# Wangkkklll/GausPcc

Hardware: AMD Instinct MI355X
Metric: Mpoints/s encode+decode @1M anchors (higher is better)
Workload: dtype f32

## Files before the change

gauspcc_amd/_lib.py:

```python
import ctypes as C
import os

_HERE = os.path.dirname(os.path.abspath(__file__))
LIB_PATH = os.environ.get("GAUSPCC_LIB") or os.path.join(_HERE, "libgauspcc.so")

_lib = None


class GpccError(RuntimeError):
    def __init__(self, code, msg):
        super().__init__(f"libgauspcc error {code}: {msg}")
        self.code = code


class Stats(C.Structure):
    _fields_ = [
        ("num_points", C.c_int64),
        ("num_bytes", C.c_int64),
        ("num_levels", C.c_int32),
        ("flags", C.c_int32),
        ("level_nodes", C.c_int64 * 24),
        ("coded_nodes", C.c_int64),
        ("conv_pairs", C.c_int64),
        ("device_ms", C.c_double),
        ("ideal_bits", C.c_double),
    ]


class Profile(C.Structure):
    _fields_ = [("conv_ms", C.c_double), ("conv_launches", C.c_int64), ("conv_pair_jobs", C.c_int64),
                ("fused_ms", C.c_double), ("fused_launches", C.c_int64), ("fused_pair_jobs", C.c_int64)]


class Stage(C.Structure):
    _fields_ = [("name", C.c_char * 48), ("ms", C.c_double), ("bytes", C.c_double), ("brackets", C.c_int64), ("critical_ms", C.c_double)]


GSR_STATE_WORDS = 16
GPCC_TRAIN_STATE_WORDS = 256
GSR_ALLOC = C.CFUNCTYPE(C.c_void_p, C.c_void_p, C.c_size_t)

EXPORTS = [
    "gpcc_last_error", "gpcc_version", "gpcc_ctx_create", "gpcc_ctx_destroy", "gpcc_ctx_bytes", "gpcc_ctx_set_container_version", "gpcc_raster_order", "gpcc_voxelise",
    "gpcc_model_create", "gpcc_model_destroy", "gpcc_encode", "gpcc_decode", "gpcc_decode_to", "gpcc_encode_batch", "gpcc_decode_batch", "gpcc_sort_zyx",
    "gpcc_build_octree", "gpcc_conv3d", "gpcc_head_cdf", "gpcc_rc_encode", "gpcc_rc_decode", "gpcc_memcpy_d2d",
    "gpcc_profile_enable", "gpcc_profile_get", "gpcc_profile_stages", "gpcc_debug_trace_enable", "gpcc_debug_trace_get", "gpcc_debug_capture", "gpcc_debug_capture_get", "gpcc_debug_exclusive_scan", "gpcc_debug_launches", "gpcc_device_error_check",
    "gsac_calculate_cdf", "gsac_encode", "gsac_decode", "gsac_encode_u16", "gsac_decode_u16", "gsac_encode_const", "gsac_decode_const", "gsac_host_encode_u16", "gsac_host_decode_u16", "gsac_host_encode_f32", "gsac_host_decode_f32", "gpcc_write_files", "gpcc_read_files", "gsac_encode_gaussian", "gsac_decode_gaussian", "gsac_encode_gaussian_mixed", "gsac_decode_gaussian_mixed", "gsac_calculate_cdf_mixed", "gsac_encode_gaussian_slices", "gsac_decode_gaussian_slices", "gsac_encode_gaussian_mixed_slices", "gsac_decode_gaussian_mixed_slices", "gshac_mlp2", "gshac_mlp2_act", "gsge_forward", "gsge_forward_train", "gsge_backward", "gsr_visible_filter", "gsr_forward", "gsr_forward_train", "gsr_backward", "gsnn_generate", "gsnn_forward_train", "gsnn_backward",
    "gpcc_train_frame", "gpcc_train_frame_nodes", "gpcc_train_weights", "gpcc_train_conv", "gpcc_train_wgrad",
    "gpcc_knn", "gpcc_scatter_max", "gpcc_grow_voxels",
    "gsr_ssim_forward", "gsr_ssim_backward",
    "gsac_rate_forward", "gsac_rate_backward",
]


def lib():
    global _lib
    if _lib is not None:
        return _lib
    if not os.path.exists(LIB_PATH):
        raise ImportError(
            f"{LIB_PATH} is missing: build it with `python -c 'import __graft_entry__ as g; g.build()'` "
            "(make -C gauspcc_amd/csrc). gauspcc_amd has no CPU fallback."
        )
    import torch

    L = C.CDLL(LIB_PATH)
    vp, i64, i32, u16 = C.c_void_p, C.c_int64, C.c_int, C.c_uint16
    L.gpcc_last_error.restype = C.c_char_p
    L.gpcc_ctx_create.argtypes = [i32, C.POINTER(vp)]
    L.gpcc_ctx_destroy.argtypes = [vp]
    L.gpcc_ctx_destroy.restype = None
    L.gpcc_ctx_bytes.argtypes = [vp, C.POINTER(i64), C.POINTER(i64)]
    L.gpcc_ctx_set_container_version.argtypes = [vp, i32]
    L.gpcc_raster_order.argtypes = [vp, vp, i32, i64, vp, vp]
    L.gpcc_voxelise.argtypes = [vp, vp, i32, i64, C.c_double, C.c_double, C.c_double, i32, vp, vp]
    L.gpcc_model_create.argtypes = [vp, i32, i32, vp, C.POINTER(vp)]
    L.gpcc_model_destroy.argtypes = [vp]
    L.gpcc_model_destroy.restype = None
    L.gpcc_encode.argtypes = [vp, vp, vp, i64, i32, u16, C.POINTER(vp), C.POINTER(i64), C.POINTER(Stats), vp]
    L.gpcc_decode.argtypes = [vp, vp, vp, i64, C.POINTER(vp), C.POINTER(i64), C.POINTER(u16), C.POINTER(Stats), vp]
    L.gpcc_encode_batch.argtypes = [vp, vp, C.POINTER(vp), C.POINTER(i64), i32, i32, C.POINTER(u16), C.POINTER(vp), C.POINTER(i64), C.POINTER(Stats), C.POINTER(i32), vp]
    L.gpcc_decode_batch.argtypes = [vp, vp, C.POINTER(vp), C.POINTER(i64), i32, C.POINTER(vp), C.POINTER(i64), C.POINTER(i64), C.POINTER(u16), C.POINTER(Stats), C.POINTER(i32), vp]
    L.gpcc_decode_to.argtypes = [vp, vp, vp, i64, vp, i64, C.POINTER(i64), C.POINTER(u16), C.POINTER(Stats), vp]
    L.gpcc_sort_zyx.argtypes = [vp, vp, i64, vp, vp]
    L.gpcc_build_octree.argtypes = [vp, vp, i64, C.POINTER(i32), C.POINTER(i64), vp, vp, i64, vp]
    L.gpcc_conv3d.argtypes = [vp, vp, i64, i32, i32, vp, vp, vp, i32, vp, C.POINTER(i64), vp]
    L.gpcc_head_cdf.argtypes = [vp, vp, i64, i32, i32, vp, vp, vp, vp, vp, vp, vp]
    L.gpcc_rc_encode.argtypes = [vp, vp, i32, vp, i64, i32, C.POINTER(vp), C.POINTER(i64), vp]
    L.gpcc_rc_decode.argtypes = [vp, vp, i32, vp, i64, i64, i32, vp, vp]
    L.gpcc_memcpy_d2d.argtypes = [vp, vp, vp, i64, vp]
    L.gpcc_profile_enable.argtypes = [vp, i32]
    L.gpcc_debug_trace_enable.argtypes = [vp, i32]
    L.gpcc_debug_trace_get.argtypes = [vp, vp, vp, i32]
    L.gpcc_debug_capture.argtypes = [vp, i32]
    L.gpcc_debug_capture_get.restype = C.c_longlong
    L.gpcc_debug_capture_get.argtypes = [vp, i32, vp, C.c_longlong]
    L.gpcc_debug_exclusive_scan.argtypes = [vp, vp, vp, vp, vp, i64, vp, vp]
    L.gpcc_debug_launches.argtypes = [i32]
    L.gpcc_device_error_check.argtypes = [vp]
    L.gpcc_debug_launches.restype = C.c_longlong
    L.gpcc_profile_get.argtypes = [vp, C.POINTER(Profile)]
    L.gpcc_profile_stages.argtypes = [vp, C.POINTER(Stage), i32, C.POINTER(i32)]
    L.gsac_calculate_cdf.argtypes = [vp, vp, vp, vp, i64, i32, i32, vp, vp]
    L.gsac_encode.argtypes = [vp, vp, vp, i32, i64, i32, C.POINTER(vp), C.POINTER(i64), C.POINTER(vp), C.POINTER(i64), vp]
    L.gsac_decode.argtypes = [vp, vp, vp, i64, vp, i32, i64, i32, vp, vp]
    L.gsac_encode_u16.argtypes = L.gsac_encode.argtypes
    L.gsac_decode_u16.argtypes = L.gsac_decode.argtypes
    L.gsac_encode_const.argtypes = L.gsac_encode.argtypes
    L.gsac_decode_const.argtypes = L.gsac_decode.argtypes
    L.gsac_host_encode_u16.argtypes = [vp, vp, i64, i32, vp, i64, C.POINTER(i64)]
    L.gsac_host_decode_u16.argtypes = [vp, vp, i64, i64, i32, vp]
    L.gsac_host_encode_f32.argtypes = L.gsac_host_encode_u16.argtypes
    L.gsac_host_decode_f32.argtypes = L.gsac_host_decode_u16.argtypes
    L.gpcc_write_files.argtypes = [vp, vp, vp, i32, i32]
    L.gpcc_read_files.argtypes = [vp, i32, i32, C.POINTER(vp), vp]
    fp = C.POINTER(C.c_float)
    L.gsac_encode_gaussian.argtypes = [vp, vp, vp, vp, vp, i64, i32, fp, fp, C.POINTER(vp), C.POINTER(i64), C.POINTER(vp), C.POINTER(i64), vp]
    L.gsac_decode_gaussian.argtypes = [vp, vp, vp, vp, i64, C.c_float, C.c_float, vp, i64, vp, i32, vp, vp]
    L.gsac_encode_gaussian_mixed.argtypes = [vp, vp, vp, vp, vp, i32, vp, i64, i32, fp, fp, C.POINTER(vp), C.POINTER(i64), C.POINTER(vp), C.POINTER(i64), vp]
    L.gsac_decode_gaussian_mixed.argtypes = [vp, vp, vp, vp, i32, vp, i64, C.c_float, C.c_float, vp, i64, vp, i32, vp, vp]
    L.gsac_calculate_cdf_mixed.argtypes = [vp, vp, vp, vp, i32, vp, i64, i32, i32, vp, vp]
    L.gsac_encode_gaussian_slices.argtypes = [vp, vp, vp, vp, vp, vp, i32, i32, vp, vp, C.POINTER(vp), C.POINTER(i64), C.POINTER(vp), C.POINTER(i64), vp]
    L.gsac_decode_gaussian_slices.argtypes = [vp, vp, vp, vp, vp, i32, vp, vp, vp, i64, vp, i32, vp, vp]
    L.gshac_mlp2.argtypes = [vp, vp, vp, vp, vp, vp, i64, i32, i32, i32, vp, vp]
    L.gshac_mlp2_act.argtypes = [vp, vp, vp, vp, vp, vp, i64, i32, i32, i32, i32, C.c_float, vp, vp]
    L.gsac_encode_gaussian_mixed_slices.argtypes = [vp, vp, vp, vp, vp, i32, vp, vp, i32, i32, vp, vp, C.POINTER(vp), C.POINTER(i64), C.POINTER(vp), C.POINTER(i64), vp]
    L.gsac_decode_gaussian_mixed_slices.argtypes = [vp, vp, vp, vp, i32, vp, vp, i32, vp, vp, vp, i64, vp, i32, vp, vp]
    L.gsge_forward.argtypes = [vp, vp, vp, vp, vp, vp, i64, i32, i32, i32, i32, vp, vp, vp]
    L.gsge_forward_train.argtypes = [vp, vp, vp, vp, vp, vp, i64, i32, i32, i32, i32, vp, vp, vp, vp]
    L.gsge_backward.argtypes = [vp, vp, vp, vp, vp, vp, i64, vp, vp, i64, i32, i32, i32, i32, vp, vp, GSR_ALLOC, vp, vp]
    f32 = C.c_float
    L.gsr_visible_filter.argtypes = [vp, i32, i32, i32, vp, vp, f32, vp, vp, vp, vp, f32, f32, i32, vp, vp]
    L.gsr_forward.argtypes = [vp, i32, vp, i32, i32, vp, vp, vp, vp, f32, vp, vp, vp, vp, f32, f32, i32, vp, vp, C.POINTER(i64), vp]
    L.gsr_forward_train.argtypes = [vp, i32, vp, i32, i32, vp, vp, vp, vp, f32, vp, vp, vp, vp, f32, f32, i32, vp, vp, GSR_ALLOC, vp,
                                    C.POINTER(C.c_uint64), C.POINTER(i64), vp]
    L.gsr_backward.argtypes = [vp, C.POINTER(C.c_uint64), i32, vp, i32, i32, vp, vp, vp, vp, f32, vp, vp, vp, vp, f32, f32, vp, vp, GSR_ALLOC, vp,
                               vp, vp, vp, vp, vp, vp, vp, vp]
    L.gsnn_generate.argtypes = [vp, i64, vp, i32, i32, vp, vp, vp, vp, vp, vp, vp, vp, vp, vp, vp, vp, C.POINTER(i64), vp]
    L.gsnn_forward_train.argtypes = [vp, i64, i32, i32, vp, vp, vp, vp, vp, vp, vp, i32, vp, vp, vp, vp, vp, vp, vp, GSR_ALLOC, vp, C.POINTER(vp),
                                     C.POINTER(i64), vp]
    L.gsnn_backward.argtypes = [vp, i64, i32, i32, vp, vp, vp, vp, vp, vp, vp, i32, vp, vp, vp, vp, vp, vp, vp, vp, vp, vp, vp, vp, vp, GSR_ALLOC, vp, vp]
    st = C.POINTER(C.c_uint64)
    L.gpcc_train_frame.argtypes = [vp, vp, i64, i32, GSR_ALLOC, vp, st, C.POINTER(i32), C.POINTER(i64), vp]
    L.gpcc_train_frame_nodes.argtypes = [vp, st, vp, vp, vp, vp, vp]
    L.gpcc_train_weights.argtypes = [vp, vp, i32, i32, i32, vp, vp]
    L.gpcc_train_conv.argtypes = [vp, st, i32, vp, vp, vp, i32, vp, vp]
    L.gpcc_train_wgrad.argtypes = [vp, st, i32, vp, vp, GSR_ALLOC, vp, vp, vp]
    L.gpcc_knn.argtypes = [vp, vp, i64, i32, vp, vp, vp, GSR_ALLOC, vp, vp]
    L.gpcc_scatter_max.argtypes = [vp, vp, vp, i64, i64, i64, i32, vp, vp, GSR_ALLOC, vp, vp]
    L.gpcc_grow_voxels.argtypes = [vp, vp, i64, vp, vp, i64, i64, vp, i64, f32, f32, C.POINTER(i64), GSR_ALLOC, vp, vp]
    L.gsr_ssim_forward.argtypes = [vp, vp, vp, i64, i64, i64, i64, i32, fp, i32, vp, vp, vp, C.c_double, vp, i32, GSR_ALLOC, vp, vp]
    L.gsr_ssim_backward.argtypes = [vp, vp, vp, i64, i64, i64, i64, i32, fp, i32, vp, i32, vp, f32, vp, f32, vp, vp, vp]
    pp, ip, f64 = C.POINTER(vp), C.POINTER(i32), C.c_double
# ... 10 lines not shown
```

gauspcc_amd/csrc/api.hip:

```cpp
#include <algorithm>

#include "fused.hpp"
#include "network.hpp"
#include "octree.hpp"
#include "primitives.hpp"
#include "rangecoder_dev.hpp"

using namespace gpcc;

namespace gpcc {
thread_local char g_err[512] = "";
thread_local long long g_launches = 0;
}

extern "C" const char *gpcc_last_error(void) { return gpcc::g_err; }
extern "C" int gpcc_version(void) { return 100; }

extern "C" int gpcc_ctx_create(int device, gpcc_ctx **out)
{
    if (!out) return fail(GPCC_ERR_ARG, "null argument");
    int count = 0;
    HIP_TRY(hipGetDeviceCount(&count));
    if (device < 0 || device >= count) return fail(GPCC_ERR_ARG, "device %d not present (%d visible)", device, count);
    HIP_TRY(hipSetDevice(device));
    hipDeviceProp_t prop;
    HIP_TRY(hipGetDeviceProperties(&prop, device));
    if (strncmp(prop.gcnArchName, "gfx950", 6) != 0) return fail(GPCC_ERR_ARG, "libgauspcc is built for gfx950 (MI355X); device %d is %s", device, prop.gcnArchName);
    gpcc_ctx *c = new gpcc_ctx();
    c->device = device;
    *out = c;
    return GPCC_OK;
}

extern "C" void gpcc_ctx_destroy(gpcc_ctx *c)
{
    if (!c) return;
    (void)hipSetDevice(c->device);
    for (hipEvent_t e : c->prof.pool) (void)hipEventDestroy(e);
    if (c->side) { (void)hipStreamSynchronize(c->side); (void)hipStreamDestroy(c->side); (void)hipStreamSynchronize(c->xfer); (void)hipStreamDestroy(c->xfer); (void)hipEventDestroy(c->ev_main); (void)hipEventDestroy(c->ev_side); (void)hipEventDestroy(c->ev_bytes); (void)hipEventDestroy(c->ev_tables); }
    if (c->arena.base) (void)hipFree(c->arena.base);
    if (c->conv_products) (void)hipFree(c->conv_products);
    fused_ctx_release(c);
    if (c->fused_state) (void)hipFree(c->fused_state);
    for (auto &ss : c->scan_states) if (ss.status) (void)hipFree(ss.status);
    if (c->dev_err) (void)hipHostFree(c->dev_err);
    if (c->hbytes.p) (void)hipHostFree(c->hbytes.p);
    if (c->dbg_dev) (void)hipFree(c->dbg_dev);
    for (auto &e : c->dbg_caps) if (e.dev) (void)hipFree(e.dev);
    if (c->hstage.p) (void)hipHostFree(c->hstage.p);
    if (c->hcoder.p) (void)hipHostFree(c->hcoder.p);
    if (c->hbatch.p) (void)hipHostFree(c->hbatch.p);
    delete c;
}

extern "C" int gpcc_device_error_check(gpcc_ctx *ctx)
{
    if (!ctx) return fail(GPCC_ERR_ARG, "null argument");
    return device_error_check(ctx);
}

extern "C" long long gpcc_debug_launches(int reset)
{
    const long long v = gpcc::g_launches;
    if (reset) gpcc::g_launches = 0;
    return v;
}

extern "C" int gpcc_ctx_set_container_version(gpcc_ctx *c, int version)
{
    if (!c) return fail(GPCC_ERR_ARG, "null argument");
    if (version != 3 && version != 4) return fail(GPCC_ERR_ARG, "container version must be 3 or 4");
    c->container_version = version;
    return GPCC_OK;
}

extern "C" int gpcc_ctx_bytes(const gpcc_ctx *c, int64_t *device_bytes, int64_t *pinned_bytes)
{
    if (!c) return fail(GPCC_ERR_ARG, "null argument");
    size_t d = c->arena.cap + c->conv_products_cap * sizeof(float) + (c->dbg_dev ? 8 * (size_t)4096 : 0);
    d += c->scan_states.size() * (8 * (size_t)65536 + 256);
    if (c->fused_state) d += 2 * 3456 + 128;
    for (const auto &e : c->dbg_caps) d += e.cap;
    if (device_bytes) *device_bytes = (int64_t)d;
    if (pinned_bytes) *pinned_bytes = (int64_t)(c->hbytes.cap + c->hstage.cap + c->hbatch.cap + c->hcoder.cap);
    return GPCC_OK;
}

namespace gpcc {
constexpr int DBG_MAX = 4096;
__global__ __launch_bounds__(256) void k_dbg_sum(const uint32_t *__restrict__ p, size_t words, unsigned long long *__restrict__ out)
{
    unsigned long long a = 0;
    for (size_t i = (size_t)blockIdx.x * 256 + threadIdx.x; i < words; i += (size_t)gridDim.x * 256) a += (unsigned long long)p[i] * (2ull * i + 1ull);
    atomicAdd(out, a);
}
int dbg_mark(gpcc_ctx *ctx, hipStream_t st, int tag, const void *p, size_t bytes)
{
    if (!ctx || !ctx->dbg_on || (int)ctx->dbg_tags.size() >= DBG_MAX) return GPCC_OK;
    const size_t words = bytes / 4;
    unsigned long long *slot = ctx->dbg_dev + ctx->dbg_tags.size();
    HIP_TRY(hipMemsetAsync(slot, 0, 8, st));
    if (words) k_dbg_sum<<<(unsigned)std::min<size_t>(1024, (words + 255) / 256), 256, 0, st>>>(static_cast<const uint32_t *>(p), words, slot);
    LAUNCH_CHECK();
    ctx->dbg_tags.push_back(tag);
    if (ctx->dbg_capture_tag_mod >= 0 && tag % 100 == ctx->dbg_capture_tag_mod && bytes) {
        gpcc_ctx::DbgCap *c = nullptr;
        for (auto &e : ctx->dbg_caps) if (e.tag == tag) c = &e;
        if (!c) { ctx->dbg_caps.push_back(gpcc_ctx::DbgCap{tag, nullptr, 0, 0}); c = &ctx->dbg_caps.back(); }
        if (c->cap < bytes) {
            if (c->dev) HIP_TRY(hipFree(c->dev));
            c->dev = nullptr; c->cap = 0;
            HIP_TRY(hipMalloc(&c->dev, bytes));
            c->cap = bytes;
        }
        c->bytes = bytes;
        HIP_TRY(hipMemcpyAsync(c->dev, p, bytes, hipMemcpyDeviceToDevice, st));
    }
    return GPCC_OK;
// ... 608 lines not shown
```

gauspcc_amd/csrc/codec.hip:

```cpp
#include <algorithm>
#include <chrono>

#include <functional>
#include "hostcoder.hpp"
#include "codec_shared.hpp"
#include "container.hpp"
#include "rangecoder_dev.hpp"

using namespace gpcc;

namespace {

constexpr int ENC_RETRY_SMALLER_CHUNKS = -1000;
constexpr int DEC_RETRY_UNFUSED = -1001;

__global__ __launch_bounds__(256) void k_set_pos(SetLevels S, int64_t nC, uint32_t *__restrict__ pos_out, uint32_t *__restrict__ slots_out)
{
    const int64_t i = (int64_t)blockIdx.x * 256 + threadIdx.x;
    if (i >= nC) return;
    int d = 1;
    for (int q = 2; q < S.L; ++q) d = i >= (int64_t)S.cbase[q] ? q : d;
    pos_out[i] = S.lohi_base[d] + rc_interleaved(S.m2r[d][i - S.cbase[d]], S.clog[d], S.nch[d]);
    slots_out[i] = S.slots[d];
}
// ... 712 lines not shown
    }
    return GPCC_OK;
}

}

static size_t arena_scaled(size_t want)
{
    static const double scale = [] { const char *e = getenv("GAUSPCC_ARENA_SCALE"); const double v = e ? atof(e) : 1.0; return v > 0.0 ? v : 1.0; }();
    return scale == 1.0 ? want : std::max<size_t>((size_t)((double)want * scale), (size_t)1 << 20);
}

extern "C" int gpcc_encode(gpcc_ctx *ctx, const gpcc_model *m, const int32_t *xyz_dev, int64_t n, int chunk_log2, uint16_t posq_f16,
                           const uint8_t **bytes_out, int64_t *nbytes_out, gpcc_stats *stats, void *stream)
{
    if (!ctx || !m || !xyz_dev || !bytes_out || !nbytes_out) return fail(GPCC_ERR_ARG, "null argument");
    if (chunk_log2 != 0 && (chunk_log2 < 6 || chunk_log2 > 14)) return fail(GPCC_ERR_ARG, "chunk_log2 must be 0 or 6..14");
    HIP_TRY(hipSetDevice(ctx->device));
    hipStream_t st = (hipStream_t)stream;
    const auto t0 = std::chrono::steady_clock::now();
    size_t want = arena_scaled(arena_estimate(n, m->K));
    int rc = GPCC_OK;
    for (int attempt = 0; attempt < 6; ++attempt) {
        GP_TRY(ctx->arena.reserve(want));
        rc = encode_body(ctx, m, xyz_dev, n, chunk_log2, posq_f16, bytes_out, nbytes_out, stats, st);
        if (rc == ENC_RETRY_SMALLER_CHUNKS) {
            HIP_TRY(hipStreamSynchronize(st));
            if (chunk_log2 <= 6) { rc = GPCC_ERR_ARG; break; }
            chunk_log2 -= 1; attempt -= 1;
            continue;
        }
        if (rc != GPCC_ERR_NOMEM) break;
        HIP_TRY(hipStreamSynchronize(st));
        want *= 2;
    }
    if (rc == GPCC_OK && stats) stats->device_ms = std::chrono::duration<double, std::milli>(std::chrono::steady_clock::now() - t0).count();
    if (const int de = device_error_check(ctx)) rc = de;
    return rc;
}

static int decode_entry(gpcc_ctx *ctx, const gpcc_model *m, const uint8_t *bytes, int64_t nbytes, const int32_t **xyz_dev_out,
                        int64_t *n_out, uint16_t *posq_f16_out, gpcc_stats *stats, void *stream, int32_t *out_user, int64_t out_cap)
{
    HIP_TRY(hipSetDevice(ctx->device));
    hipStream_t st = (hipStream_t)stream;
    const auto t0 = std::chrono::steady_clock::now();
    size_t want = arena_estimate(std::max<int64_t>(nbytes, 1 << 16), m->K);
    int64_t nodes = 0, nmax = 0, npts = 0;
    const int pre = container_precheck(bytes, nbytes, &nodes, &nmax, &npts);
    if (pre < 0) return pre;
    if (pre > 0) {
        const int L = bytes[6];
        want = (size_t)nmax * 2600 + (size_t)nodes * (size_t)(4 * 125 + m->K * 81 / 16 + 96) + (size_t)npts * 32 + (size_t)nbytes + ((size_t)48 << 20);
        if (fused_enabled()) {
            int64_t nf = 0;
            for (int d = 0; d < L; ++d) { const int64_t v = get32(bytes + 8 + 4 * d); if (fused_level_ok(v, m->k)) nf = std::max(nf, v); }
            want += (size_t)nf * (size_t)m->K * (128 + 10 + 9) + ((size_t)4 << 20);
        }
    }
    want = arena_scaled(want);
    ctx->fused_note_decode();
    int rc = GPCC_OK;
    const int32_t *xyz = nullptr;
    for (int attempt = 0; attempt < 6; ++attempt) {
        GP_TRY(ctx->arena.reserve(want));
        rc = decode_body(ctx, m, bytes, nbytes, &xyz, n_out, posq_f16_out, stats, st, out_user, out_cap);
        if (rc == DEC_RETRY_UNFUSED) {
            static const bool loud = getenv("GAUSPCC_FUSED_QUIET") == nullptr;
            if (loud) fprintf(stderr, "[gauspcc] a persistent small-level launch timed out on device %d; the launch-per-layer path serves this context's next %d decodes\n", ctx->device, ctx->fused_rearm_after);
            attempt -= 1;
            continue;
        }
        if (rc != GPCC_ERR_NOMEM) break;
        HIP_TRY(hipStreamSynchronize(st));
        want *= 2;
    }
    if (rc == GPCC_OK && xyz_dev_out) *xyz_dev_out = xyz;
    if (rc == GPCC_OK && stats) stats->device_ms = std::chrono::duration<double, std::milli>(std::chrono::steady_clock::now() - t0).count();
    if (const int de = device_error_check(ctx)) rc = de;
    return rc;
}

extern "C" int gpcc_decode(gpcc_ctx *ctx, const gpcc_model *m, const uint8_t *bytes, int64_t nbytes, const int32_t **xyz_dev_out,
                           int64_t *n_out, uint16_t *posq_f16_out, gpcc_stats *stats, void *stream)
{
    if (!ctx || !m || !bytes || !xyz_dev_out || !n_out || !posq_f16_out) return fail(GPCC_ERR_ARG, "null argument");
    return decode_entry(ctx, m, bytes, nbytes, xyz_dev_out, n_out, posq_f16_out, stats, stream, nullptr, 0);
}

extern "C" int gpcc_decode_to(gpcc_ctx *ctx, const gpcc_model *m, const uint8_t *bytes, int64_t nbytes, int32_t *xyz_dev, int64_t capacity_points,
                              int64_t *n_out, uint16_t *posq_f16_out, gpcc_stats *stats, void *stream)
{
    if (!ctx || !m || !bytes || !xyz_dev || capacity_points < 0 || !n_out || !posq_f16_out) return fail(GPCC_ERR_ARG, "null argument");
    return decode_entry(ctx, m, bytes, nbytes, nullptr, n_out, posq_f16_out, stats, stream, xyz_dev, capacity_points);
}
```

gauspcc_amd/csrc/codec_batch.hip:

```cpp
#include <algorithm>
#include <chrono>
#include <functional>

#include "codec_shared.hpp"
#include "container.hpp"
#include "forest.hpp"
#include "rangecoder_dev.hpp"

using namespace gpcc;

extern "C" int gpcc_encode(gpcc_ctx *ctx, const gpcc_model *m, const int32_t *xyz_dev, int64_t n, int chunk_log2, uint16_t posq_f16, const uint8_t **bytes_out, int64_t *nbytes_out,
                           gpcc_stats *stats, void *stream);
extern "C" int gpcc_decode_to(gpcc_ctx *ctx, const gpcc_model *m, const uint8_t *bytes, int64_t nbytes, int32_t *xyz_dev, int64_t capacity_points, int64_t *n_out,
                              uint16_t *posq_f16_out, gpcc_stats *stats, void *stream);

namespace {

constexpr int BATCH_SOLO = -2001;
constexpr int BATCH_RETRY_UNFUSED = -2002;

struct FPosArgs {
    int L;
    uint32_t cbase[MAXLV];
    const uint32_t *m2r[MAXLV];
// ... 807 lines not shown
            if (r1 != GPCC_OK) {
                char msg[400]; snprintf(msg, sizeof msg, "%s", g_err);
                return fail(r1, "scene %d: %s", q, msg);
            }
            offsets_out[q] = (int64_t)blob.size();
            blob.insert(blob.end(), b, b + nb);
            if (stats) stats[q] = s1;
        }
        offsets_out[nscenes] = (int64_t)blob.size();
        GP_TRY(ctx->hbytes.reserve(blob.size() + 16));
        memcpy(ctx->hbytes.p, blob.data(), blob.size());
        *bytes_out = ctx->hbytes.p;
        rc = GPCC_OK;
    }
    if (rc == GPCC_OK && stats) stats[0].device_ms = std::chrono::duration<double, std::milli>(std::chrono::steady_clock::now() - t0).count();
    if (const int de = device_error_check(ctx)) rc = de;
    return rc;
}

extern "C" int gpcc_decode_batch(gpcc_ctx *ctx, const gpcc_model *m, const uint8_t *const *bytes, const int64_t *nbytes, int nscenes, int32_t *const *xyz_dev,
                                 const int64_t *capacity_points, int64_t *n_out, uint16_t *posq_f16_out, gpcc_stats *stats, int *batched_out, void *stream)
{
    if (!ctx || !m || !bytes || !nbytes || !xyz_dev || !capacity_points || !n_out || !posq_f16_out || nscenes < 1) return fail(GPCC_ERR_ARG, "null argument");
    for (int q = 0; q < nscenes; ++q) if (!bytes[q] || !xyz_dev[q] || capacity_points[q] < 0 || nbytes[q] < 0) return fail(GPCC_ERR_ARG, "scene %d: null argument", q);
    HIP_TRY(hipSetDevice(ctx->device));
    hipStream_t st = (hipStream_t)stream;
    const auto t0 = std::chrono::steady_clock::now();
    int rc = BATCH_SOLO;
    if (batched_out) *batched_out = 0;
    static const bool never = env_int("GAUSPCC_BATCH", 1) == 0;
    if (nscenes <= FOREST_MAX_SCENES && !never) {
        int64_t nodes = 0, nmax_sum[MAXLV] = {0}, total_bytes = 0, npts = 0;
        bool ok = true;
        for (int q = 0; q < nscenes && ok; ++q) {
            const uint8_t *b = bytes[q];
            total_bytes += nbytes[q];
            if (!(nbytes[q] >= 8 && b[0] == 0xFF && b[1] == 0xFF && b[6] >= 1 && b[6] <= 21 && nbytes[q] >= 12 + 4 * (int64_t)b[6])) { ok = false; break; }
            const int L = b[6];
            int64_t prev = 0, mine = 0;
            for (int d = 0; d < L; ++d) {
                const int64_t v = get32(b + 8 + 4 * d);
                if (v <= 0 || (d == 0 ? v >= 64 : v > 8 * prev)) { ok = false; break; }
                mine += v; nmax_sum[d] += v; prev = v;
            }
            if (!ok) break;
            const int64_t np = get32(b + 8 + 4 * L);
            if (np < 1 || np > 8 * prev || mine > (nbytes[q] << 13)) { ok = false; break; }
            nodes += mine; npts += np;
        }
        if (ok) {
            ctx->fused_note_decode();
            int64_t nmax = 0;
            for (int d = 0; d < MAXLV; ++d) nmax = std::max(nmax, nmax_sum[d]);
            size_t want = arena_scaled_b((size_t)nmax * 2700 + (size_t)nodes * (size_t)(4 * 125 + m->K * 81 / 16 + 96) + (size_t)npts * 32 + (size_t)total_bytes + (size_t)nscenes * 65536 + ((size_t)48 << 20));
            if (fused_enabled()) {
                int64_t nf = 0;
                for (int d = 0; d < MAXLV; ++d) if (nmax_sum[d] > 0 && fused_level_ok(nmax_sum[d], m->k)) nf = std::max(nf, nmax_sum[d]);
                want += (size_t)nf * (size_t)m->K * (128 + 10 + 9) + ((size_t)4 << 20);
            }
            for (int attempt = 0; attempt < 6; ++attempt) {
                GP_TRY(ctx->arena.reserve(want));
                rc = decode_batch_body(ctx, m, bytes, nbytes, nscenes, xyz_dev, capacity_points, n_out, posq_f16_out, stats, st);
                if (rc == BATCH_RETRY_UNFUSED) {
                    static const bool loud = getenv("GAUSPCC_FUSED_QUIET") == nullptr;
                    if (loud) fprintf(stderr, "[gauspcc] a persistent small-level launch timed out on device %d; the launch-per-layer path serves this context's next %d decodes\n", ctx->device, ctx->fused_rearm_after);
                    attempt -= 1;
                    continue;
                }
                if (rc != GPCC_ERR_NOMEM) break;
                HIP_TRY(hipStreamSynchronize(st));
                want *= 2;
            }
            if (rc == GPCC_OK && batched_out) *batched_out = 1;
        }
    }
    if (rc == BATCH_SOLO) {
        HIP_TRY(hipStreamSynchronize(st));
        for (int q = 0; q < nscenes; ++q) {
            gpcc_stats s1; memset(&s1, 0, sizeof s1);
            const int r1 = gpcc_decode_to(ctx, m, bytes[q], nbytes[q], xyz_dev[q], capacity_points[q], &n_out[q], &posq_f16_out[q], &s1, stream);
            if (r1 != GPCC_OK) {
                char msg[400]; snprintf(msg, sizeof msg, "%s", g_err);
                return fail(r1, "scene %d: %s", q, msg);
            }
            if (stats) stats[q] = s1;
        }
        rc = GPCC_OK;
    }
    if (rc == GPCC_OK && stats) stats[0].device_ms = std::chrono::duration<double, std::milli>(std::chrono::steady_clock::now() - t0).count();
    if (const int de = device_error_check(ctx)) rc = de;
    return rc;
}
```

gauspcc_amd/csrc/network.hpp:

```cpp
#pragma once
#include "common.hpp"

struct gpcc_model {
    int C = 32, k = 5, K = 125;
    float *slab = nullptr;
    const float *prior_emb = nullptr;
    const float *conv[18] = {0};
    const float *temb = nullptr;
    const float *hw1[4] = {0}, *hb1[4] = {0}, *hw2[4] = {0}, *hb2[4] = {0};
    const float *hfrag[4] = {0};
    const float *semb[3] = {0};
};

namespace gpcc {

__host__ __device__ __forceinline__ int phys_of(int c)
{
    const int kk = c >> 2, g = c & 3;
    return kk < 4 ? 4 * g + kk : 16 + 4 * g + (kk - 4);
}
__host__ __device__ __forceinline__ int logical_of(int p)
{
    const int kk = 4 * (p >> 4) + (p & 3), g = (p & 15) >> 2;
    return 4 * kk + g;
// ... 17 lines not shown
                for (int lane = 0; lane < 64; ++lane)
                    for (int r = 0; r < 4; ++r) {
                        const int m = lane & 15;
                        out[((((size_t)o * 2 + hh) * 2 + q) * 64 + lane) * 4 + r] = W[((size_t)o * 32 + (4 * (4 * q + r) + (lane >> 4))) * 32 + 16 * hh + 4 * (m & 3) + (m >> 2)];
                    }
}

constexpr int STAGE_M[4] = {2, 2, 4, 16};

struct ConvJob {
    const float *in;
    const float *w;
    const float *res;
    float *out;
};
struct ConvBatch { ConvJob job[4]; int C = 0; };

constexpr int CONV_R_MAX = 255;
constexpr int CONV_HDR_PAD = 48;
struct ConvTiles {
    int32_t *tj = nullptr;
    uint8_t *tr = nullptr;
    uint32_t *toc = nullptr;
    uint32_t *first = nullptr;
    uint32_t *order = nullptr;
    int64_t nblk = 0;
    int R = CONV_R_MAX;
    int H = CONV_R_MAX;
    int K = 0;
    int paired = 0;
    const uint8_t *pflag = nullptr;
    int nlv = 0;
    uint32_t lv_blk0[MAXLV + 1] = {0};
    uint32_t lv_row0[MAXLV] = {0};
    uint32_t lv_rows[MAXLV] = {0};
};
int conv_pick_rows(int64_t n, int k = 5);
bool conv_is_coop(int64_t n, int R);
int conv_pick_height(int64_t n, int R);

struct Level;
struct TileLevel { const Level *lv; const Level *par; const int32_t *cell_par; int32_t *cell_own; };
struct TilePool {
    int32_t *tj = nullptr; uint8_t *tr = nullptr; uint32_t *toc = nullptr; uint32_t *first = nullptr;
    int64_t nblk = 0;
    int R = 0, H = 0, K = 0, nlv = 0, paired = 0;
    uint8_t *pflag = nullptr;
    uint32_t lv_blk0[MAXLV + 1] = {0}, lv_rows[MAXLV] = {0};
    double alg_bytes = 0.0;
};
int cell_map_entries(int k);
int tiles_build(gpcc_ctx *ctx, hipStream_t st, const TileLevel *lv, int nlv, int k, int R, int H, TilePool *pool, unsigned long long *pairs_dev);
int tiles_dense_map(hipStream_t st, const Level *par, const int32_t *cell_par, const Level *chi, int32_t *cell_own, int k, int32_t *nbr, uint16_t *rk, uint32_t *rowcnt);
int tiles_view(gpcc_ctx *ctx, hipStream_t st, const TilePool &pool, int l0, int l1, const int64_t *row_base, ConvTiles *T);

int sparse_conv(gpcc_ctx *ctx, int level, hipStream_t st, const ConvBatch &jobs, int njobs, const ConvTiles &T, int64_t n, int relu);
int conv_chain_begin(gpcc_ctx *ctx, hipStream_t st);
int conv_chain_end(gpcc_ctx *ctx, hipStream_t st);
int prof_collect(gpcc_ctx *ctx, const unsigned long long *pairs_per_level, int nlevels);

int embed_occ(hipStream_t st, const float *emb, const uint8_t *occ, int64_t n, float *out, int C = 32);
int child_features(hipStream_t st, const float *F, const uint32_t *parent, const uint64_t *rkey_c, const float *temb, int64_t n, float *out, int C = 32);
int stage_inputs_gt(hipStream_t st, const float *X, const float *const emb[3], const uint8_t *occ, int64_t n, float *const out[3], int C = 32);
int stage_input_dec(hipStream_t st, const float *X, const float *emb, const uint8_t *const sym_r[3], const uint32_t *m2r, int stage, int64_t n, float *out, int C = 32);

constexpr int HEAD_FRAG_FLOATS = 1024 + 512 + 32 + 16;
struct HeadArgs {
    const float *x; int64_t n; int stage_m;
    const float *w1, *b1, *w2, *b2;
    const float *frag;
    const uint32_t *m2r; const uint8_t *occ; int stage;
    uint32_t *lohi; uint16_t *cdf; float *prob; int mode;
    int chunk_log2; uint32_t nch;
    const uint32_t *pos; const uint32_t *slots;
    double *bits;
    int C;
};
int head_cdf(hipStream_t st, const HeadArgs &a);

int assemble_occ(hipStream_t st, const uint8_t *const sym_r[4], const uint32_t *m2r, int64_t n, uint8_t *occ);

int any_embed_occ(hipStream_t st, const float *emb, const uint8_t *occ, int64_t n, float *out, int C);
int any_child_features(hipStream_t st, const float *F, const uint32_t *parent, const uint64_t *rkey_c, const float *temb, int64_t n, float *out, int C);
int any_stage_inputs_gt(hipStream_t st, const float *X, const float *const emb[3], const uint8_t *occ, int64_t n, float *const out[3], int C);
int any_stage_input_dec(hipStream_t st, const float *X, const float *emb, const uint8_t *const sym_r[3], const uint32_t *m2r, int stage, int64_t n, float *out, int C);
int any_sparse_conv(hipStream_t st, const ConvBatch &jobs, int njobs, const ConvTiles &T, int64_t n, int relu, int C);
int any_head_cdf(hipStream_t st, const HeadArgs &a, int C);

int rows_permute(hipStream_t st, const float *in, float *out, int64_t n, int to_physical);

}
```

gauspcc_amd/csrc/tiles.hip:

```cpp
#include "network.hpp"
#include "octree.hpp"
#include "primitives.hpp"

namespace gpcc {

namespace {

struct LevelTilesArgs {
    const uint64_t *rkey_c; const uint32_t *parent_c; int64_t nc;
    const int32_t *cell_p; int64_t np; const uint8_t *occ_p; const uint32_t *cstart_p;
    int H;
    int paired;
    uint8_t *pflag;
    uint32_t blk0;
    int32_t *cell_c;
    uint32_t *per_block;
    unsigned long long *pairs;
    uint8_t *cnt_oq;
    const uint32_t *first;
    int32_t *tj; uint8_t *tr; uint32_t *toc;
    int32_t *nbr; uint16_t *rk; uint32_t *rowcnt;
};

struct WaveMap {
// ... 328 lines not shown
        uint32_t inc = nt;
#pragma unroll
        for (int d = 1; d < 64; d <<= 1) {
            const uint32_t v = (uint32_t)__shfl_up((int)inc, d, 64);
            if (lane >= d) inc += v;
        }
        const uint32_t tb = carry + inc - nt;
        for (uint32_t i = 0; i < nt; ++i) toc[tb + i] = (uint32_t)o | ((tot > 16u * i ? min(16u, tot - 16u * i) : 0u) << 16);
        for (uint32_t p = tot; p < nt * 16u; ++p) { tj[(size_t)tb * 16 + p] = 0; tr[(size_t)tb * 16 + p] = 0; }
        carry += (uint32_t)__shfl((int)inc, 63, 64);
    }
}

template <int KS, bool FILL>
int launch_level(hipStream_t st, const LevelTilesArgs &a, bool tail)
{
    const int H = a.H;
    const bool multi = H == 16 || H == 32;
    const int nq = H > 64 ? (H + 63) / 64 : 1;
    const unsigned grid = multi ? (unsigned)cdiv(a.nc, 64) : (unsigned)(cdiv(a.nc, H) * nq);
    if (nq > 1) k_chunk_tiles<KS, FILL, true><<<grid, 64, 0, st>>>(a);
    else k_chunk_tiles<KS, FILL, false><<<grid, 64, 0, st>>>(a);
    LAUNCH_CHECK();
    if (nq > 1 && tail) {
        const int nblk = (int)cdiv(a.nc, H);
        if (!FILL) k_block_sum<<<(unsigned)cdiv(nblk, 4), 256, 0, st>>>(a.cnt_oq, a.blk0, nblk, KS * KS * KS, a.per_block, a.paired, a.pflag);
        else k_tile_words<<<(unsigned)cdiv(nblk, 4), 256, 0, st>>>(a.cnt_oq, a.first, a.blk0, nblk, KS * KS * KS, a.tj, a.tr, a.toc, a.pflag);
        LAUNCH_CHECK();
    }
    return GPCC_OK;
}

template <bool FILL>
int run_level(hipStream_t st, const Level *par, const int32_t *cell_par, const Level *chi, int k, LevelTilesArgs a, bool tail = true)
{
    a.rkey_c = chi->rkey; a.parent_c = chi->parent; a.nc = chi->n;
    if (a.H < 16 || a.H > CONV_R_MAX) return fail(GPCC_ERR_ARG, "internal: block height %d", a.H);
    if (!par) {
        if (chi->n >= 64) return fail(GPCC_ERR_ARG, "internal: base level with %lld nodes", (long long)chi->n);
        const int Hb = std::min(a.H, 64);
        k_base_tiles<FILL><<<(unsigned)cdiv(chi->n, (Hb == 16 || Hb == 32) ? 64 : Hb), 64, 0, st>>>(a, k);
        LAUNCH_CHECK();
        return GPCC_OK;
    }
    a.cell_p = cell_par; a.np = par->n; a.occ_p = par->occ; a.cstart_p = par->cstart;
    switch (k) {
    case 3: return launch_level<3, FILL>(st, a, tail);
    case 5: return launch_level<5, FILL>(st, a, tail);
    case 7: return launch_level<7, FILL>(st, a, tail);
    default: return fail(GPCC_ERR_ARG, "kernel_size must be 3, 5 or 7");
    }
}

__global__ __launch_bounds__(64) void k_fold_pairs(const unsigned long long *__restrict__ spread, int nlv, unsigned long long *__restrict__ pairs)
{
    for (int l = 0; l < nlv; ++l) {
        unsigned long long v = spread[l * 64 + threadIdx.x];
#pragma unroll
        for (int d = 32; d >= 1; d >>= 1) v += __shfl_xor(v, d, 64);
        if (threadIdx.x == 0) pairs[l] += v;
    }
}

__global__ __launch_bounds__(256) void k_order_keys(const uint32_t *__restrict__ first, uint32_t b0, int nblk, uint64_t *__restrict__ key, uint32_t *__restrict__ idx)
{
    const int b = blockIdx.x * 256 + threadIdx.x;
    if (b >= nblk) return;
    key[b] = 0xFFFFull - (uint64_t)min(first[b0 + b + 1] - first[b0 + b], 0xFFFFu);
    idx[b] = b0 + (uint32_t)b;
}

__global__ __launch_bounds__(64) void k_pad_tiles(const uint32_t *__restrict__ total, int32_t *__restrict__ tj, uint32_t *__restrict__ tr4, uint32_t *__restrict__ toc)
{
    const uint32_t t = *total;
    for (int i = threadIdx.x; i < CONV_HDR_PAD * 16; i += 64) tj[(size_t)t * 16 + i] = 0;
    for (int i = threadIdx.x; i < CONV_HDR_PAD * 4; i += 64) tr4[(size_t)t * 4 + i] = 0;
    for (int i = threadIdx.x; i < CONV_HDR_PAD; i += 64) toc[t + i] = 0;
}

}

int cell_map_entries(int k) { const int PW = 2 * ((k / 2 + 1) / 2) + 1; return PW * PW * PW; }

int tiles_build(gpcc_ctx *ctx, hipStream_t st, const TileLevel *lv, int nlv, int k, int R, int H, TilePool *pool, unsigned long long *pairs_dev)
{
    if (nlv < 1 || nlv > MAXLV) return fail(GPCC_ERR_ARG, "internal: %d levels", nlv);
    const int K = k * k * k;
    pool->R = R; pool->H = H; pool->K = K; pool->nlv = nlv;
    int64_t nblk = 0;
    for (int l = 0; l < nlv; ++l) {
        if (lv[l].lv->n >= (int64_t)1 << 31) return fail(GPCC_ERR_ARG, "level too large");
        pool->lv_blk0[l] = (uint32_t)nblk;
        pool->lv_rows[l] = (uint32_t)lv[l].lv->n;
        nblk += cdiv(lv[l].lv->n, H);
    }
    if (nblk >= (int64_t)1 << 31) return fail(GPCC_ERR_ARG, "too many blocks");
    pool->lv_blk0[nlv] = (uint32_t)nblk;
    pool->nblk = nblk;
    TAKE(first, uint32_t, nblk + 1);
    pool->first = first;
    LevelTilesArgs a = {};
    static const bool pair_on = dev_env_int("GAUSPCC_CONV_PAIR", 1) != 0;
    static const int pair_min = 150;
    pool->paired = (H > 64 && R == CONV_R_MAX && pair_on) ? std::max(pair_min, 1) : 0;
    pool->pflag = nullptr;
    unsigned long long *spread = nullptr;
    {
        const size_t b_sp = pairs_dev ? 8 * (size_t)nlv * 64 : 0;
        const size_t b_cq = H > 64 ? (((size_t)nblk * K * 4 + 15) & ~(size_t)15) : 0;
        const size_t b_pf = pool->paired ? (((size_t)nblk + 15) & ~(size_t)15) : 0;
        if (b_sp + b_cq + b_pf) {
            TAKE(z, unsigned long long, (b_sp + b_cq + b_pf) / 8);
            uint8_t *zb = reinterpret_cast<uint8_t *>(z);
            HIP_TRY(hipMemsetAsync(zb, 0, b_sp + b_cq + b_pf, st));
            if (b_sp) spread = z;
            if (b_cq) a.cnt_oq = zb + b_sp;
            if (b_pf) pool->pflag = zb + b_sp + b_cq;
        }
    }
    a.H = H; a.paired = pool->paired; a.pflag = pool->pflag; a.per_block = first;
    const bool batch = nlv > 1;
    for (int l = 1; l < nlv; ++l) if (!lv[l].par) return fail(GPCC_ERR_ARG, "internal: level %d of a tile pool has no parent", l);
    const int lp = lv[0].par ? 0 : 1;
    for (int l = 0; l < nlv; ++l) {
        a.blk0 = pool->lv_blk0[l]; a.cell_c = lv[l].cell_own; a.pairs = spread ? spread + (size_t)l * 64 : nullptr;
        GP_TRY(run_level<false>(st, lv[l].par, lv[l].cell_par, lv[l].lv, k, a, !batch));
    }
    if (batch && H > 64 && lp < nlv) {
        const uint32_t b1 = pool->lv_blk0[lp];
        k_block_sum<<<(unsigned)cdiv(nblk - b1, 4), 256, 0, st>>>(a.cnt_oq, b1, (int)(nblk - b1), K, a.per_block, a.paired, a.pflag);
        LAUNCH_CHECK();
    }
    if (spread) { k_fold_pairs<<<1, 64, 0, st>>>(spread, nlv, pairs_dev); LAUNCH_CHECK(); }
    GP_TRY(exclusive_scan_u32(ctx, st, first, first, nblk, first + nblk));
    {
        const int NPc = cell_map_entries(k);
        double b = 0.0;
        for (int l = 0; l < nlv; ++l)
            b += (double)lv[l].lv->n * (12 + (lv[l].cell_own ? 4.0 * NPc : 0.0)) + (lv[l].par ? (double)lv[l].par->n * 9.0 * NPc : 0.0);
        pool->alg_bytes = b;
    }
    int64_t cap;
    int64_t rows_total = 0;
    for (int l = 0; l < nlv; ++l) rows_total += lv[l].lv->n;
    if (H <= 16) cap = nblk * K + CONV_HDR_PAD;
    else if (H <= 64 && H % 16 == 0 && conv_is_coop(rows_total, R)) cap = nblk * K * (H / 16) + CONV_HDR_PAD;
    else {
        {
            uint32_t total = 0;
            HIP_TRY(hipMemcpyAsync(&total, first + nblk, 4, hipMemcpyDeviceToHost, st));
            HIP_TRY(hipStreamSynchronize(st));
            cap = (int64_t)total + CONV_HDR_PAD;
            pool->alg_bytes += 84.0 * total;
        }
    }
    if (cap >= (int64_t)1 << 28) return fail(GPCC_ERR_ARG, "too many conv tiles (%lld): clouds beyond ~10^8 points need 64-bit tile addressing", (long long)cap);
    TAKE(tj, int32_t, cap * 16);
    TAKE(tr, uint8_t, cap * 16);
    TAKE(toc, uint32_t, cap);
    pool->tj = tj; pool->tr = tr; pool->toc = toc;
    k_pad_tiles<<<1, 64, 0, st>>>(first + nblk, tj, reinterpret_cast<uint32_t *>(tr), toc);
    LAUNCH_CHECK();
    a.first = first; a.tj = tj; a.tr = tr; a.toc = toc; a.cell_c = nullptr; a.pairs = nullptr;
    if (!batch) {
        a.blk0 = pool->lv_blk0[0];
        GP_TRY(run_level<true>(st, lv[0].par, lv[0].cell_par, lv[0].lv, k, a));
        return GPCC_OK;
    }
    if (lp == 1) { a.blk0 = pool->lv_blk0[0]; GP_TRY(run_level<true>(st, nullptr, nullptr, lv[0].lv, k, a)); }
    {
        SetTilesArgs S = {};
        S.common = a;
        const bool multi = H == 16 || H == 32;
        const int nq = H > 64 ? (H + 63) / 64 : 1;
        uint32_t g = 0;
        for (int l = lp; l < nlv; ++l) {
            auto &d = S.lv[l - lp];
            d.rkey_c = lv[l].lv->rkey; d.parent_c = lv[l].lv->parent; d.nc = lv[l].lv->n; d.cell_p = lv[l].cell_par; d.np = lv[l].par->n;
            d.occ_p = lv[l].par->occ; d.cstart_p = lv[l].par->cstart; d.blk0 = pool->lv_blk0[l];
            S.g0[l - lp] = g;
            g += multi ? (uint32_t)cdiv(d.nc, 64) : (uint32_t)(cdiv(d.nc, H) * nq);
        }
        S.nlv = nlv - lp; S.g0[S.nlv] = g;
        switch (k) {
        case 3: if (nq > 1) k_fill_tiles_set<3, true><<<g, 64, 0, st>>>(S); else k_fill_tiles_set<3, false><<<g, 64, 0, st>>>(S); break;
        case 5: if (nq > 1) k_fill_tiles_set<5, true><<<g, 64, 0, st>>>(S); else k_fill_tiles_set<5, false><<<g, 64, 0, st>>>(S); break;
        case 7: if (nq > 1) k_fill_tiles_set<7, true><<<g, 64, 0, st>>>(S); else k_fill_tiles_set<7, false><<<g, 64, 0, st>>>(S); break;
        default: return fail(GPCC_ERR_ARG, "kernel_size must be 3, 5 or 7");
        }
        LAUNCH_CHECK();
        if (nq > 1) {
            const uint32_t b1 = pool->lv_blk0[lp];
            k_tile_words<<<(unsigned)cdiv(nblk - b1, 4), 256, 0, st>>>(a.cnt_oq, a.first, b1, (int)(nblk - b1), K, tj, tr, toc, a.pflag);
            LAUNCH_CHECK();
        }
    }
    return GPCC_OK;
}

int tiles_dense_map(hipStream_t st, const Level *par, const int32_t *cell_par, const Level *chi, int32_t *cell_own, int k, int32_t *nbr, uint16_t *rk, uint32_t *rowcnt)
{
    if (!par) return fail(GPCC_ERR_ARG, "internal: dense map of a level without a parent");
    LevelTilesArgs a = {};
    a.H = 64; a.blk0 = 0; a.cell_c = cell_own; a.nbr = nbr; a.rk = rk; a.rowcnt = rowcnt;
    a.rkey_c = chi->rkey; a.parent_c = chi->parent; a.nc = chi->n;
    a.cell_p = cell_par; a.np = par->n; a.occ_p = par->occ; a.cstart_p = par->cstart;
    const unsigned grid = (unsigned)cdiv(chi->n, 64);
    switch (k) {
    case 3: k_chunk_dense<3><<<grid, 64, 0, st>>>(a); break;
    case 5: k_chunk_dense<5><<<grid, 64, 0, st>>>(a); break;
    case 7: k_chunk_dense<7><<<grid, 64, 0, st>>>(a); break;
    default: return fail(GPCC_ERR_ARG, "kernel_size must be 3, 5 or 7");
    }
    LAUNCH_CHECK();
// ... 33 lines not shown
```

include/gauspcc.h:

```cpp
#ifndef GAUSPCC_H
#define GAUSPCC_H

#include <stddef.h>
#include <stdint.h>

#ifdef __cplusplus
extern "C" {
#endif

#define GPCC_API __attribute__((visibility("default")))

typedef enum {
    GPCC_OK = 0,
    GPCC_ERR_HIP = -1,
    GPCC_ERR_ARG = -2,
    GPCC_ERR_RANGE = -3,
    GPCC_ERR_DUPLICATE = -4,
    GPCC_ERR_FORMAT = -5,
    GPCC_ERR_NOMEM = -6
} gpcc_status;

typedef enum { GPCC_F32 = 0, GPCC_F64 = 1, GPCC_I32 = 2, GPCC_I64 = 3 } gpcc_dtype;

typedef struct gpcc_ctx gpcc_ctx;
typedef struct gpcc_model gpcc_model;

GPCC_API const char *gpcc_last_error(void);
GPCC_API int gpcc_version(void);

GPCC_API int gpcc_ctx_create(int device, gpcc_ctx **out);
GPCC_API void gpcc_ctx_destroy(gpcc_ctx *ctx);
GPCC_API int gpcc_ctx_set_container_version(gpcc_ctx *ctx, int version);
GPCC_API int gpcc_ctx_bytes(const gpcc_ctx *ctx, int64_t *device_bytes, int64_t *pinned_bytes);

GPCC_API long long gpcc_debug_launches(int reset);

GPCC_API int gpcc_device_error_check(gpcc_ctx *ctx);

GPCC_API int gpcc_raster_order(gpcc_ctx *ctx, const void *xyz_dev, int dtype, int64_t n,
                      int64_t *perm_out_dev, void *stream);

#define GPCC_VOX_SCALE 1
#define GPCC_VOX_POSQ 2
GPCC_API int gpcc_voxelise(gpcc_ctx *ctx, const void *xyz_dev, int dtype, int64_t n, double d1, double add, double d2, int flags,
                  int32_t *out_dev, void *stream);

typedef enum {
    GPCC_T_PRIOR_EMB = 0,
    GPCC_T_CONV0 = 1,
    GPCC_T_TEMB = 19,
    GPCC_T_HW1 = 20,
    GPCC_T_HB1 = 24,
    GPCC_T_HW2 = 28,
    GPCC_T_HB2 = 32,
    GPCC_T_SEMB = 36,
    GPCC_T_COUNT = 39
} gpcc_tensor_id;

GPCC_API int gpcc_model_create(gpcc_ctx *ctx, int channels, int kernel_size, const float *const *tensors,
                      gpcc_model **out);
GPCC_API void gpcc_model_destroy(gpcc_model *m);

#define GPCC_STATS_IDEAL_BITS 1
typedef struct {
    int64_t num_points;
    int64_t num_bytes;
    int32_t num_levels;
    int32_t flags;
    int64_t level_nodes[24];
    int64_t coded_nodes;
    int64_t conv_pairs;
    double device_ms;
    double ideal_bits;
} gpcc_stats;

GPCC_API int gpcc_encode(gpcc_ctx *ctx, const gpcc_model *m, const int32_t *xyz_dev, int64_t n,
                int chunk_log2, uint16_t posq_f16, const uint8_t **bytes_out, int64_t *nbytes_out,
                gpcc_stats *stats, void *stream);

GPCC_API int gpcc_decode(gpcc_ctx *ctx, const gpcc_model *m, const uint8_t *bytes, int64_t nbytes,
                const int32_t **xyz_dev_out, int64_t *n_out, uint16_t *posq_f16_out,
                gpcc_stats *stats, void *stream);

GPCC_API int gpcc_decode_to(gpcc_ctx *ctx, const gpcc_model *m, const uint8_t *bytes, int64_t nbytes,
                int32_t *xyz_dev, int64_t capacity_points, int64_t *n_out, uint16_t *posq_f16_out,
                gpcc_stats *stats, void *stream);

GPCC_API int gpcc_encode_batch(gpcc_ctx *ctx, const gpcc_model *m, const int32_t *const *xyz_dev, const int64_t *n, int nscenes,
// ... 211 lines not shown
```

Before: 21.18.

## Bound conv tile pool on host to skip device readback sync, fold pair reduction

Adds a host-side upper bound on the conv tile count for single-level, moderately tall tile heights, so the tile pool can be sized without copying the scanned total back and synchronising the stream. The pair-count fold kernel is merged into the padding kernel to save a launch. Arena sizing in decode paths is raised to cover the larger worst-case pools. This trades extra device memory for removing a host-device round trip on the critical path, and adds a debug export for checking the bound.

```diff
diff --git a/gauspcc_amd/_lib.py b/gauspcc_amd/_lib.py
--- a/gauspcc_amd/_lib.py
+++ b/gauspcc_amd/_lib.py
@@ -44,7 +44,7 @@
     "gpcc_last_error", "gpcc_version", "gpcc_ctx_create", "gpcc_ctx_destroy", "gpcc_ctx_bytes", "gpcc_ctx_set_container_version", "gpcc_raster_order", "gpcc_voxelise",
     "gpcc_model_create", "gpcc_model_destroy", "gpcc_encode", "gpcc_decode", "gpcc_decode_to", "gpcc_encode_batch", "gpcc_decode_batch", "gpcc_sort_zyx",
     "gpcc_build_octree", "gpcc_conv3d", "gpcc_head_cdf", "gpcc_rc_encode", "gpcc_rc_decode", "gpcc_memcpy_d2d",
-    "gpcc_profile_enable", "gpcc_profile_get", "gpcc_profile_stages", "gpcc_debug_trace_enable", "gpcc_debug_trace_get", "gpcc_debug_capture", "gpcc_debug_capture_get", "gpcc_debug_exclusive_scan", "gpcc_debug_launches", "gpcc_device_error_check",
+    "gpcc_profile_enable", "gpcc_profile_get", "gpcc_profile_stages", "gpcc_debug_trace_enable", "gpcc_debug_trace_get", "gpcc_debug_capture", "gpcc_debug_capture_get", "gpcc_debug_exclusive_scan", "gpcc_debug_launches", "gpcc_debug_tile_pool_bound", "gpcc_device_error_check",
     "gsac_calculate_cdf", "gsac_encode", "gsac_decode", "gsac_encode_u16", "gsac_decode_u16", "gsac_encode_const", "gsac_decode_const", "gsac_host_encode_u16", "gsac_host_decode_u16", "gsac_host_encode_f32", "gsac_host_decode_f32", "gpcc_write_files", "gpcc_read_files", "gsac_encode_gaussian", "gsac_decode_gaussian", "gsac_encode_gaussian_mixed", "gsac_decode_gaussian_mixed", "gsac_calculate_cdf_mixed", "gsac_encode_gaussian_slices", "gsac_decode_gaussian_slices", "gsac_encode_gaussian_mixed_slices", "gsac_decode_gaussian_mixed_slices", "gshac_mlp2", "gshac_mlp2_act", "gsge_forward", "gsge_forward_train", "gsge_backward", "gsr_visible_filter", "gsr_forward", "gsr_forward_train", "gsr_backward", "gsnn_generate", "gsnn_forward_train", "gsnn_backward",
     "gpcc_train_frame", "gpcc_train_frame_nodes", "gpcc_train_weights", "gpcc_train_conv", "gpcc_train_wgrad",
     "gpcc_knn", "gpcc_scatter_max", "gpcc_grow_voxels",
@@ -99,6 +99,8 @@
     L.gpcc_debug_launches.argtypes = [i32]
     L.gpcc_device_error_check.argtypes = [vp]
     L.gpcc_debug_launches.restype = C.c_longlong
+    L.gpcc_debug_tile_pool_bound.argtypes = [C.c_longlong, i32, C.POINTER(C.c_int), C.POINTER(C.c_int)]
+    L.gpcc_debug_tile_pool_bound.restype = C.c_longlong
     L.gpcc_profile_get.argtypes = [vp, C.POINTER(Profile)]
     L.gpcc_profile_stages.argtypes = [vp, C.POINTER(Stage), i32, C.POINTER(i32)]
     L.gsac_calculate_cdf.argtypes = [vp, vp, vp, vp, i64, i32, i32, vp, vp]
diff --git a/gauspcc_amd/csrc/api.hip b/gauspcc_amd/csrc/api.hip
--- a/gauspcc_amd/csrc/api.hip
+++ b/gauspcc_amd/csrc/api.hip
@@ -64,6 +64,15 @@
     const long long v = gpcc::g_launches;
     if (reset) gpcc::g_launches = 0;
     return v;
+}
+
+extern "C" long long gpcc_debug_tile_pool_bound(long long n, int kernel_size, int *height_out, int *paired_out)
+{
+    if (n <= 0 || (kernel_size != 3 && kernel_size != 5 && kernel_size != 7)) return -1;
+    const int R = gpcc::conv_pick_rows(n, kernel_size), H = gpcc::conv_pick_height(n, R);
+    if (height_out) *height_out = H;
+    if (paired_out) *paired_out = (H > 64 && R == gpcc::CONV_R_MAX) ? 1 : 0;
+    return (long long)gpcc::tiles_pool_bound(n, kernel_size);
 }
 
 extern "C" int gpcc_ctx_set_container_version(gpcc_ctx *c, int version)
diff --git a/gauspcc_amd/csrc/codec.hip b/gauspcc_amd/csrc/codec.hip
--- a/gauspcc_amd/csrc/codec.hip
+++ b/gauspcc_amd/csrc/codec.hip
@@ -788,6 +788,7 @@
     if (pre > 0) {
         const int L = bytes[6];
         want = (size_t)nmax * 2600 + (size_t)nodes * (size_t)(4 * 125 + m->K * 81 / 16 + 96) + (size_t)npts * 32 + (size_t)nbytes + ((size_t)48 << 20);
+        for (int d = 0; d < L; ++d) { const int64_t v = get32(bytes + 8 + 4 * d); if (v > 0) want += 84 * (size_t)tiles_pool_bound(v, m->k); }
         if (fused_enabled()) {
             int64_t nf = 0;
             for (int d = 0; d < L; ++d) { const int64_t v = get32(bytes + 8 + 4 * d); if (fused_level_ok(v, m->k)) nf = std::max(nf, v); }
diff --git a/gauspcc_amd/csrc/codec_batch.hip b/gauspcc_amd/csrc/codec_batch.hip
--- a/gauspcc_amd/csrc/codec_batch.hip
+++ b/gauspcc_amd/csrc/codec_batch.hip
@@ -883,7 +883,9 @@
             ctx->fused_note_decode();
             int64_t nmax = 0;
             for (int d = 0; d < MAXLV; ++d) nmax = std::max(nmax, nmax_sum[d]);
-            size_t want = arena_scaled_b((size_t)nmax * 2700 + (size_t)nodes * (size_t)(4 * 125 + m->K * 81 / 16 + 96) + (size_t)npts * 32 + (size_t)total_bytes + (size_t)nscenes * 65536 + ((size_t)48 << 20));
+            size_t pool_b = 0;
+            for (int d = 0; d < MAXLV; ++d) if (nmax_sum[d] > 0) pool_b += 84 * (size_t)tiles_pool_bound(nmax_sum[d], m->k);
+            size_t want = arena_scaled_b(pool_b + (size_t)nmax * 2700 + (size_t)nodes * (size_t)(4 * 125 + m->K * 81 / 16 + 96) + (size_t)npts * 32 + (size_t)total_bytes + (size_t)nscenes * 65536 + ((size_t)48 << 20));
             if (fused_enabled()) {
                 int64_t nf = 0;
                 for (int d = 0; d < MAXLV; ++d) if (nmax_sum[d] > 0 && fused_level_ok(nmax_sum[d], m->k)) nf = std::max(nf, nmax_sum[d]);
diff --git a/gauspcc_amd/csrc/network.hpp b/gauspcc_amd/csrc/network.hpp
--- a/gauspcc_amd/csrc/network.hpp
+++ b/gauspcc_amd/csrc/network.hpp
@@ -93,6 +93,7 @@
 int cell_map_entries(int k);
 int tiles_build(gpcc_ctx *ctx, hipStream_t st, const TileLevel *lv, int nlv, int k, int R, int H, TilePool *pool, unsigned long long *pairs_dev);
 int tiles_dense_map(hipStream_t st, const Level *par, const int32_t *cell_par, const Level *chi, int32_t *cell_own, int k, int32_t *nbr, uint16_t *rk, uint32_t *rowcnt);
+int64_t tiles_pool_bound(int64_t n, int k);
 int tiles_view(gpcc_ctx *ctx, hipStream_t st, const TilePool &pool, int l0, int l1, const int64_t *row_base, ConvTiles *T);
 
 int sparse_conv(gpcc_ctx *ctx, int level, hipStream_t st, const ConvBatch &jobs, int njobs, const ConvTiles &T, int64_t n, int relu);
diff --git a/gauspcc_amd/csrc/tiles.hip b/gauspcc_amd/csrc/tiles.hip
--- a/gauspcc_amd/csrc/tiles.hip
+++ b/gauspcc_amd/csrc/tiles.hip
@@ -404,16 +404,6 @@
     }
 }
 
-__global__ __launch_bounds__(64) void k_fold_pairs(const unsigned long long *__restrict__ spread, int nlv, unsigned long long *__restrict__ pairs)
-{
-    for (int l = 0; l < nlv; ++l) {
-        unsigned long long v = spread[l * 64 + threadIdx.x];
-#pragma unroll
-        for (int d = 32; d >= 1; d >>= 1) v += __shfl_xor(v, d, 64);
-        if (threadIdx.x == 0) pairs[l] += v;
-    }
-}
-
 __global__ __launch_bounds__(256) void k_order_keys(const uint32_t *__restrict__ first, uint32_t b0, int nblk, uint64_t *__restrict__ key, uint32_t *__restrict__ idx)
 {
     const int b = blockIdx.x * 256 + threadIdx.x;
@@ -422,14 +412,38 @@
     idx[b] = b0 + (uint32_t)b;
 }
 
-__global__ __launch_bounds__(64) void k_pad_tiles(const uint32_t *__restrict__ total, int32_t *__restrict__ tj, uint32_t *__restrict__ tr4, uint32_t *__restrict__ toc)
+__global__ __launch_bounds__(64) void k_pad_tiles(const uint32_t *__restrict__ total, int32_t *__restrict__ tj, uint32_t *__restrict__ tr4, uint32_t *__restrict__ toc,
+                                                  const unsigned long long *__restrict__ spread, int nlv, unsigned long long *__restrict__ pairs)
 {
     const uint32_t t = *total;
     for (int i = threadIdx.x; i < CONV_HDR_PAD * 16; i += 64) tj[(size_t)t * 16 + i] = 0;
     for (int i = threadIdx.x; i < CONV_HDR_PAD * 4; i += 64) tr4[(size_t)t * 4 + i] = 0;
     for (int i = threadIdx.x; i < CONV_HDR_PAD; i += 64) toc[t + i] = 0;
-}
-
+    if (!spread) return;
+    for (int l = 0; l < nlv; ++l) {
+        unsigned long long v = spread[l * 64 + threadIdx.x];
+#pragma unroll
+        for (int d = 32; d >= 1; d >>= 1) v += __shfl_xor(v, d, 64);
+        if (threadIdx.x == 0) pairs[l] += v;
+    }
+}
+
+}
+
+constexpr int POOL_BOUND_MAX_H = 128;
+static int64_t pool_bound_tiles(int64_t nblk, int K, int R, int H, int64_t rows, int paired, bool single)
+{
+    if (H <= 16) return nblk * K;
+    if (H <= 64 && H % 16 == 0 && conv_is_coop(rows, R)) return nblk * K * (H / 16);
+    if (single && H <= POOL_BOUND_MAX_H && nblk <= 1024) return nblk * K * (int64_t)run_tiles((uint32_t)H, paired);
+    return 0;
+}
+
+int64_t tiles_pool_bound(int64_t n, int k)
+{
+    const int R = conv_pick_rows(n, k), H = conv_pick_height(n, R);
+    const int paired = (H > 64 && R == CONV_R_MAX) ? 1 : 0;
+    return pool_bound_tiles(cdiv(n, H), k * k * k, R, H, n, paired, true);
 }
 
 int cell_map_entries(int k) { const int PW = 2 * ((k / 2 + 1) / 2) + 1; return PW * PW * PW; }
@@ -483,7 +497,6 @@
         k_block_sum<<<(unsigned)cdiv(nblk - b1, 4), 256, 0, st>>>(a.cnt_oq, b1, (int)(nblk - b1), K, a.per_block, a.paired, a.pflag);
         LAUNCH_CHECK();
     }
-    if (spread) { k_fold_pairs<<<1, 64, 0, st>>>(spread, nlv, pairs_dev); LAUNCH_CHECK(); }
     GP_TRY(exclusive_scan_u32(ctx, st, first, first, nblk, first + nblk));
     {
         const int NPc = cell_map_entries(k);
@@ -495,23 +508,20 @@
     int64_t cap;
     int64_t rows_total = 0;
     for (int l = 0; l < nlv; ++l) rows_total += lv[l].lv->n;
-    if (H <= 16) cap = nblk * K + CONV_HDR_PAD;
-    else if (H <= 64 && H % 16 == 0 && conv_is_coop(rows_total, R)) cap = nblk * K * (H / 16) + CONV_HDR_PAD;
+    if (const int64_t bound = pool_bound_tiles(nblk, K, R, H, rows_total, pool->paired, nlv == 1)) cap = bound + CONV_HDR_PAD;
     else {
-        {
-            uint32_t total = 0;
-            HIP_TRY(hipMemcpyAsync(&total, first + nblk, 4, hipMemcpyDeviceToHost, st));
-            HIP_TRY(hipStreamSynchronize(st));
-            cap = (int64_t)total + CONV_HDR_PAD;
-            pool->alg_bytes += 84.0 * total;
-        }
+        uint32_t total = 0;
+        HIP_TRY(hipMemcpyAsync(&total, first + nblk, 4, hipMemcpyDeviceToHost, st));
+        HIP_TRY(hipStreamSynchronize(st));
+        cap = (int64_t)total + CONV_HDR_PAD;
+        pool->alg_bytes += 84.0 * total;
     }
     if (cap >= (int64_t)1 << 28) return fail(GPCC_ERR_ARG, "too many conv tiles (%lld): clouds beyond ~10^8 points need 64-bit tile addressing", (long long)cap);
     TAKE(tj, int32_t, cap * 16);
     TAKE(tr, uint8_t, cap * 16);
     TAKE(toc, uint32_t, cap);
     pool->tj = tj; pool->tr = tr; pool->toc = toc;
-    k_pad_tiles<<<1, 64, 0, st>>>(first + nblk, tj, reinterpret_cast<uint32_t *>(tr), toc);
+    k_pad_tiles<<<1, 64, 0, st>>>(first + nblk, tj, reinterpret_cast<uint32_t *>(tr), toc, spread, nlv, pairs_dev);
     LAUNCH_CHECK();
     a.first = first; a.tj = tj; a.tr = tr; a.toc = toc; a.cell_c = nullptr; a.pairs = nullptr;
     if (!batch) {
diff --git a/include/gauspcc.h b/include/gauspcc.h
--- a/include/gauspcc.h
+++ b/include/gauspcc.h
@@ -34,6 +34,7 @@
 GPCC_API int gpcc_ctx_bytes(const gpcc_ctx *ctx, int64_t *device_bytes, int64_t *pinned_bytes);
 
 GPCC_API long long gpcc_debug_launches(int reset);
+GPCC_API long long gpcc_debug_tile_pool_bound(long long n, int kernel_size, int *height_out, int *paired_out);
 
 GPCC_API int gpcc_device_error_check(gpcc_ctx *ctx);
 
```

Result: no change. 20.98 (-1.0%).
